# hdm0922/PathTracerDemo

Hardware: AMD Instinct MI355X
Metric: Msamples/sec at 1920x1080, 1 spp ReSTIR DI; per-pixel L2 vs WebGPU ref (higher is better)
Workload: dtype f32; 1 GPU; c3_interior_32 reuse 1920x1080, 1 spp/frame (configs[2]); frame=1920x1080, band_rows_per_gpu=1080, parallelism=row-bands x1

## Files before the change

### pathtracerdemo_amd/csrc/ptx_api.cpp

```cpp
#include <hip/hip_runtime.h>

#include <algorithm>
#include <cmath>
#include <cstdarg>
#include <cstdlib>
#include <cstdio>
#include <cstring>
#include <new>
#include <string>
#include <unordered_map>
#include <vector>

#include "ptx_internal.h"

namespace ptx {


[[maybe_unused]] static const char *const kShippedKnobs[] = {"COMM_TIMEOUT_S", "DEBUG_FILL", "HALO_PROXY_US"};
#if defined(PTX_WG_TIMES)
static const char *const kBuildKind = "wgt";
#elif defined(PTX_AB_BUILD)
static const char *const kBuildKind = "ab";
#else
static const char *const kBuildKind = "product";
// ... 37 lines not shown
            return end - pos == n ? 1 : std::atoi(ab.c_str() + pos + n + 1);
        pos = end + 1;
    }
    return dflt;
}

int fail(ptx_handle *h, int code, const char *fmt, ...) {
    if (h) {
        char buf[512];
        va_list ap;
        va_start(ap, fmt);
        vsnprintf(buf, sizeof buf, fmt, ap);
        va_end(ap);
        h->err = buf;
        gbuf_key_drop_all(h);
    }
    return code;
}
void gbuf_key_of(const ptx_handle *h, uint32_t *key) {
    static_assert(ptx_handle::kGbufKeyWords == 2 + 19 + 8 + 3, "G-buffer key words");
    key[0] = h->uniform[0];
    key[1] = h->uniform[1];
    std::memcpy(key + 2, h->uniform + 4, 19 * sizeof(uint32_t));
    std::memcpy(key + 21, h->uniform + 24, 8 * sizeof(uint32_t));
    key[29] = h->cfg.row_begin;
    key[30] = h->band_h;
    key[31] = h->halo_top;
}
void gbuf_key_drop(ptx_handle *h) { h->cur().gbuf_key_valid = false; }
void gbuf_key_drop_all(ptx_handle *h) {
    for (auto &c : h->ctx) c.gbuf_key_valid = false;
}
static bool gbuf_kept(const ptx_handle *h) {
    static const bool keep_on = ab_knob("GBUF_KEEP", 1) != 0;
    if (!keep_on || !h->cur().gbuf_key_valid || h->gbuf_exposed) return false;
    uint32_t key[ptx_handle::kGbufKeyWords];
    gbuf_key_of(h, key);
    return std::memcmp(key, h->cur().gbuf_key, sizeof key) == 0;
}
void free_buf(DevBuf &b) {
    if (b.p) (void)hipFree(b.p);
    b.p = nullptr;
    b.bytes = 0;
}
static hipError_t memset_sync(ptx_handle *h, void *p, int value, size_t bytes) {
    hipError_t e = hipMemsetAsync(p, value, bytes, h->cur().stream);
// ... 421 lines not shown
}

static size_t px_with_halo(const ptx_handle *h) {
    return (size_t)(h->halo_top + h->band_h + h->halo_bot) * h->cfg.width;
}
static uint32_t gi_job_slots(const ptx_handle *h) { return std::max(2u * h->reuse_neighbors, kGiMotionSlots); }
int reuse_buffers(ptx_handle *h) {
    const size_t njobs = (size_t)h->band_h * h->cfg.width *
                         (h->cfg.pipeline == PTX_PIPELINE_RESTIR_GI ? gi_job_slots(h) : reuse_jobs_per_px(h));
    if (h->cfg.pipeline == PTX_PIPELINE_RESTIR_GI) return alloc_buf(h, h->d_jres, njobs * 4u);
    if (int rc = alloc_buf(h, h->d_jstate, njobs * 6u * 16u)) return rc;
    if (int rc = alloc_buf(h, h->cur().nbr, px_with_halo(h) * 16u)) return rc;
    const size_t npix = (size_t)h->band_h * h->cfg.width;
    if (int rc = alloc_buf(h, h->cur().tjstate, npix * kMotionJobs * 6u * 16u)) return rc;
    if (int rc = alloc_buf(h, h->cur().tjres, npix * kMotionJobs * 16u)) return rc;
    return alloc_buf(h, h->d_jres, njobs * 16u);
}
static ReuseArgs reuse_args(ptx_handle *h, int pass) {
    ReuseArgs A{};
    A.gbuf = gbuf_band(h);
    A.cur = res_band(h);
    A.hist = hist_band(h);
    const bool temporal = pass == PTX_PASS_TEMPORAL;
    A.jstate = (float4 *)(temporal ? h->cur().tjstate.p : h->d_jstate.p);
    A.jres = (float4 *)(temporal ? h->cur().tjres.p : h->d_jres.p);
    A.jpp = temporal ? 1u : 2u * h->reuse_neighbors;
    A.njobs = h->band_h * h->cfg.width * A.jpp;
    static const bool planes = ab_knob("JOB_PLANES", 1) != 0;
    A.jpx = planes ? 1u : A.jpp;
    A.jslot = planes ? h->band_h * h->cfg.width : 1u;
    A.radius = h->reuse_radius;
    A.neighbors = h->reuse_neighbors;
    A.cap = h->temporal_cap;
    A.hist_valid = h->hist_valid && !h->hist_moved ? 1u : 0u;
    A.use_init = (pass == PTX_PASS_TEMPORAL && h->cur().init_state_valid) ? 1u : 0u;
    A.nbr_out = (uint4 *)h->cur().nbr.p + (size_t)h->halo_top * h->cfg.width;
    A.nbr = A.nbr_out;
    A.surf = h->cur().surf.p ? (const uint4 *)h->cur().surf.p + 2u * (size_t)h->halo_top * h->cfg.width : nullptr;
    static const bool fold_off = ab_knob("FOLD_LAST_STEP", 1) == 0;
    A.fold_last = ((pass == PTX_PASS_SPATIAL || pass == PTX_PASS_TEMPORAL) && !fold_off) ? 1u : 0u;
    A.ray_cap = (uint32_t)std::min<size_t>(h->cur().wave_ray_cap, 0xffffffffu);
    return A;
}

void mat4_inverse(const float *mf, float *out);
static ReuseArgs motion_args(ptx_handle *h) {
    ReuseArgs A = reuse_args(h, PTX_PASS_SPATIAL);
    A.jstate = (float4 *)h->cur().tjstate.p;
    A.jres = (float4 *)h->cur().tjres.p;
    A.jpp = kMotionJobs;
    A.njobs = h->band_h * h->cfg.width * A.jpp;
    static const bool planes = ab_knob("JOB_PLANES", 1) != 0;
    A.jpx = planes ? 1u : A.jpp;
    A.jslot = planes ? h->band_h * h->cfg.width : 1u;
    A.hist_valid = h->hist_valid ? 1u : 0u;
    A.use_init = h->cur().init_state_valid ? 1u : 0u;
    static const bool fold_on = ab_knob("FOLD_LAST_STEP", 1) != 0;
    A.fold_last = fold_on ? 1u : 0u;
    A.motion = 1u;
    std::memcpy(A.vpinv_prev, h->hist_camera, sizeof A.vpinv_prev);
    mat4_inverse(A.vpinv_prev, A.vp_prev);
    const size_t W = h->cfg.width;
    A.psurf = (const uint4 *)h->d_psurf.p + 2u * (size_t)h->halo_top * W;
    A.prev_row_lo = -(int32_t)h->halo_top;
    A.prev_row_hi = (int32_t)(h->band_h + h->halo_bot);
    A.clip = (unsigned long long *)h->d_counters.p + CNT_MOTION_CLIP;
    return A;
}

static GiArgs gi_args(ptx_handle *h, bool motion) {
    GiArgs A{};
    A.gbuf = gbuf_band(h);
    A.cur = res_band(h);
    A.hist = hist_band(h);
    A.direct = (float4 *)h->cur().direct.p;
    A.accum = (float4 *)h->d_accum.p;
    A.jray = (uint32_t *)h->d_jres.p;
    A.jpp = 2u * h->reuse_neighbors;
    static const bool planes = ab_knob("GI_JOB_PLANES", 1) != 0;
    A.jpx = planes ? 1u : A.jpp;
    A.jslot = planes ? h->band_h * h->cfg.width : 1u;
// ... 184 lines not shown
                e = wave_trace(sc, wt, r - 1, 1, h->stack_depth, st);
                event_end(t, st);
                if (e != hipSuccess) break;
            }
            if (r == nr && A.fold_last) continue;
            TimedLaunch *t = event_begin(h, PTX_STAT_WAVE_LOGIC, st);
            e = wave_reuse_round(sc, wi, 0, r, A, st);
            if (e == hipSuccess && r == 0 && halo) e = hipStreamWaitEvent(st, halo, 0);
            if (e == hipSuccess) e = wave_reuse_round(sc, we, 0, r, A, st);
            event_end(t, st);
        }
        for (const WaveBufs *ws : {&wi, &we})
            if (e == hipSuccess) e = launch_wave_seq(h, sc, *ws, PTX_PASS_FINAL, st);
    }
    if (surf_stale && e == hipSuccess) h->cur().surf_valid = true;
    return e == hipSuccess ? join_sequences(h, k) : e;
}

hipError_t launch_wave_parts(ptx_handle *h, const Scene &sc, const WaveBufs &w, const int *passes, int npasses,
                             bool summaries, const WaveBufs *then, hipEvent_t then_wait, bool keep_gbuf) {
    static const bool overlap_start = ab_knob("OVERLAP_START", 1) != 0;
    if (then && overlap_start && npasses == 2 && passes[0] == PTX_PASS_SPATIAL && passes[1] == PTX_PASS_FINAL &&
        h->cfg.pipeline == PTX_PIPELINE_RESTIR_REUSE && !summaries)
        return spatial_overlap_seq(h, sc, w, *then, then_wait);
    static const int env_k = ab_knob("WAVE_STREAMS", 0);
    static const int env_pk = ab_knob("PIPE_STREAMS", 0);
    const bool band_h = h->comm || h->halo_top || h->halo_bot || (h->cfg.flags & PTX_FLAG_HALO_SKIP);
    const int pipe_k = env_pk > 0 ? env_pk
                       : band_h || h->cfg.pipeline == PTX_PIPELINE_RESTIR_GI ||
                                 (h->cfg.pipeline == PTX_PIPELINE_RESTIR_REUSE && !reuse_static())
// ... 8 lines not shown
    k = std::max(1, std::min<int>(k, ptx_handle::kMaxSplit));
    if ((uint32_t)k > std::max(w.nseg, then ? then->nseg : 0u)) k = (int)std::max(w.nseg, then ? then->nseg : 0u);
    hipError_t e = hipSuccess;
    bool has_gbuf = false;
    for (int i = 0; i < npasses; ++i) has_gbuf |= passes[i] == PTX_PASS_GBUFFER;
    const bool skip_gbuf = has_gbuf && keep_gbuf && gbuf_kept(h);
    if (has_gbuf && !skip_gbuf) h->cur().gbuf_key_valid = false;
    for (int i = 0; i < npasses; ++i) {
        if (passes[i] == PTX_PASS_SPATIAL) {
            if (summaries && (e = spatial_summaries(h, h->cur().stream)) != hipSuccess) return e;
        } else if (passes[i] == PTX_PASS_GBUFFER && skip_gbuf) {
            continue;
        } else if (passes[i] != PTX_PASS_FINAL && passes[i] != PTX_PASS_TEMPORAL && passes[i] != kPassTemporalJobs &&
                   passes[i] != kPassTemporalCombine && !is_motion_pass(passes[i])) {
            h->cur().nbr_valid = false;
        }
    }
    bool need_surf[8] = {false};
    bool surf_ok = h->cur().surf_valid;
    for (int i = 0; i < npasses && i < 8; ++i) {
        if (passes[i] == PTX_PASS_GBUFFER) surf_ok = surf_ok && skip_gbuf;
        else if (passes[i] == PTX_PASS_INIT && w.surf) surf_ok = true;
        else if ((passes[i] == PTX_PASS_TEMPORAL || passes[i] == kPassTemporalJobs || passes[i] == PTX_PASS_SPATIAL ||
                  is_motion_pass(passes[i])) &&
                 w.surf) {
            need_surf[i] = !surf_ok;
            surf_ok = true;
        }
    }
    h->cur().surf_valid = surf_ok && w.surf;
// ... 29 lines not shown
                    e = launch_wave_seq(h, sc, part, passes[i], st);
                }
                if (e != hipSuccess) return e;
            }
        }
    }
    if ((e = join_sequences(h, k)) != hipSuccess) return e;
    if (has_gbuf && !skip_gbuf) {
        gbuf_key_of(h, h->cur().gbuf_key);
        h->cur().gbuf_key_valid = true;
    }
    for (int i = 0; i < npasses; ++i)
        if (passes[i] == PTX_PASS_TEMPORAL || passes[i] == kPassTemporalCombine || passes[i] == kPassTemporalMotion) {
            h->cur().init_state_valid = false;
            h->cur().nbr_valid = h->cfg.pipeline == PTX_PIPELINE_RESTIR_REUSE;
        }
    return hipSuccess;
}
static hipError_t launch_wave_pass(ptx_handle *h, const Scene &sc, const WaveBufs &w, int pass) {
    return launch_wave_parts(h, sc, w, &pass, 1);
}

void mark_history(ptx_handle *h) {
    std::memcpy(h->hist_camera, h->uniform + 4, sizeof h->hist_camera);
    h->hist_valid = true;
    h->hist_moved = false;
}

void mat4_inverse(const float *mf, float *out) {
    double m[16], inv[16];
// ... 181 lines not shown
        if (e == hipSuccess) e = launch_wave_parts(h, sc, w, back, 2);
        if (e == hipSuccess) mark_history(h);
    } else {
        static const int passes[3] = {PTX_PASS_GBUFFER, PTX_PASS_INIT, PTX_PASS_FINAL};
        e = launch_wave_parts(h, sc, w, passes, 3, true, nullptr, nullptr, true);
    }
    if (e != hipSuccess) return fail(h, PTX_E_HIP, "wavefront frame launch: %s", hipGetErrorString(e));
    HIP_CHECK(h, hipEventRecord(t.stop, h->cur().stream));
    t.pass = PTX_STAT_FRAME;
    t.pending = true;
    return PTX_OK;
}

static int timed_launch(ptx_handle *h, int pass) {
    if (!h->scene_loaded || !h->frame_set) return fail(h, PTX_E_INVALID, "scene and frame must be set before rendering");
    if (pass != PTX_PASS_TEMPORAL && pass != PTX_PASS_SPATIAL && pass != PTX_PASS_FINAL) h->cur().nbr_valid = false;
    if (!h->layout_valid) {
        if (int rc = build_layout(h)) return rc;
    }
    TimedLaunch &t = h->ring[h->ring_pos];
    h->ring_pos = (h->ring_pos + 1) % kEventRing;
    resolve_event(t, h);
    Scene sc = make_scene(h);
    const uint32_t fl = h->cfg.flags;
    const int variant = (fl & PTX_FLAG_SIMPLE_KERNELS) ? 2 : 3;
    WaveBufs w{};
    const bool reuse_pass = pass == PTX_PASS_TEMPORAL || pass == PTX_PASS_SPATIAL;
    if (reuse_pass && (variant != 3 || !has_reuse(h)))
        return fail(h, PTX_E_INVALID, "pass %d needs the reuse or GI pipeline (wavefront kernels)", pass);
    if (h->cfg.pipeline == PTX_PIPELINE_RESTIR_GI && pass == PTX_PASS_MCPT)
        return fail(h, PTX_E_INVALID, "the GI pipeline has no MCPT pass");
// ... 179 lines not shown
    HIP_CHECK(h, hipSetDevice(h->device));
    if (!scene || !geometry || (!accel && n_accel)) return fail(h, PTX_E_INVALID, "null scene array");
    if (int rc = quiesce(h)) return rc;
    h->scene.assign(scene, scene + n_scene);
    h->geometry.assign(geometry, geometry + n_geometry);
    h->accel.assign(accel ? accel : scene, accel ? accel + n_accel : scene);
    if (int rc = upload(h, h->d_scene, scene, n_scene * 4u)) return rc;
    if (int rc = upload(h, h->d_geometry, geometry, n_geometry * 4u)) return rc;
    h->layout_valid = false;
    h->scene_loaded = true;
    h->hist_valid = false;
    h->cur().init_state_valid = false;
    h->cur().nbr_valid = false;
    for (auto &c : h->ctx) c.surf_valid = false;
    gbuf_key_drop_all(h);
    if (h->frame_set) return build_layout(h);
    return PTX_OK;
}

int ptx_set_frame(ptx_handle *h, const uint32_t uniform[PTX_UNIFORM_WORDS]) {
    if (!h || !uniform) return PTX_E_INVALID;
    HIP_CHECK(h, hipSetDevice(h->device));
    if (uniform[0] != h->cfg.width || uniform[1] != h->cfg.height)
        return fail(h, PTX_E_INVALID, "uniform resolution %ux%u != handle %ux%u", uniform[0], uniform[1],
                    h->cfg.width, h->cfg.height);
    uint32_t key[8];
    for (int k = 0; k < 8; ++k) key[k] = uniform[24 + k];
    if (std::memcmp(key, h->layout_key, sizeof key) != 0) {
        std::memcpy(h->layout_key, key, sizeof key);
        h->layout_valid = false;
// ... 235 lines not shown
    DevBuf b;
    if (!buffer_view(h, which, b) || bytes > b.bytes)
        return fail(h, PTX_E_INVALID, "read of %zu bytes from buffer %d", bytes, which);
    if (int rc = read_to_host(h, host_dst, b.p, bytes)) return rc;
    return PTX_OK;
}

int ptx_write_buffer(ptx_handle *h, int which, const void *host_src, size_t bytes) {
    if (!h || !host_src) return PTX_E_INVALID;
    DevBuf b;
    if (!buffer_view(h, which, b) || bytes > b.bytes)
        return fail(h, PTX_E_INVALID, "write of %zu bytes to buffer %d", bytes, which);
    HIP_CHECK(h, copy_sync(h, b.p, host_src, bytes, hipMemcpyHostToDevice));
    h->cur().init_state_valid = false;
    h->cur().nbr_valid = false;
    h->cur().surf_valid = false;
    if (which == PTX_BUF_GBUFFER) gbuf_key_drop(h);
    return PTX_OK;
}

int ptx_device_pointer(ptx_handle *h, int which, void **dev_ptr, size_t *bytes) {
    if (!h || !dev_ptr) return PTX_E_INVALID;
    DevBuf b;
    if (!buffer_view(h, which, b)) return fail(h, PTX_E_INVALID, "unknown buffer %d", which);
    *dev_ptr = b.p;
    if (bytes) *bytes = b.bytes;
    if (which == PTX_BUF_GBUFFER) {
        h->gbuf_exposed = true;
        gbuf_key_drop_all(h);
    }
    return PTX_OK;
}

int ptx_present(ptx_handle *h, uint32_t canvas_w, uint32_t canvas_h, int bgra, uint8_t *out) {
    if (!h || !out) return PTX_E_INVALID;
    if (canvas_w == 0 || canvas_h == 0 || (uint64_t)canvas_w * canvas_h > (1ull << 28))
        return fail(h, PTX_E_INVALID, "ptx_present: canvas %ux%u", canvas_w, canvas_h);
    if (h->cfg.row_begin != 0 || h->band_h != h->cfg.height)
        return fail(h, PTX_E_INVALID, "ptx_present: a band handle (rows %u..%u) holds part of the texture: present the "
                                      "gathered frame on the host", h->cfg.row_begin, h->cfg.row_end);
    if (!h->d_accum.p) return fail(h, PTX_E_INVALID, "ptx_present: nothing rendered");
    HIP_CHECK(h, hipSetDevice(h->device));
    const size_t bytes = (size_t)canvas_w * canvas_h * 4u;
    if (int rc = alloc_buf(h, h->d_canvas, bytes)) return rc;
// ... 95 lines not shown
    if (h->xstream) (void)hipStreamSynchronize(h->xstream);
    comm_destroy(h);
    if (h->ctx[0].own) (void)hipStreamSynchronize(h->ctx[0].own);
    for (auto &t : h->ring) {
        if (t.start) (void)hipEventDestroy(t.start);
        if (t.stop) (void)hipEventDestroy(t.stop);
    }
    if (h->host_stage) (void)hipHostFree(h->host_stage);
    if (h->ev_present) {
        (void)hipEventSynchronize(h->ev_present);
        (void)hipEventDestroy(h->ev_present);
    }
    if (h->present_host) (void)hipHostFree(h->present_host);
    for (DevBuf *b : {&h->d_canvas, &h->d_canvas_async, &h->d_scene, &h->d_geometry, &h->d_tris, &h->d_nodes, &h->d_subs,
                      &h->d_insts, &h->d_mats, &h->d_tverts, &h->d_accum, &h->d_counters, &h->d_qrays, &h->d_qhits, &h->d_hist,
                      &h->d_jstate, &h->d_jres, &h->d_psurf, &h->d_census, &h->d_wgt})
        free_buf(*b);
    for (auto &c : h->ctx) {
        for (DevBuf *b : {&c.gbuf, &c.res, &c.direct, &c.nbr, &c.tjstate, &c.tjres, &c.surf, &c.wstate, &c.wrays, &c.wres[0],
                          &c.wres[1], &c.wres[2], &c.wact[0], &c.wact[1], &c.wctr})
            free_buf(*b);
        if (c.ev_fork) (void)hipEventDestroy(c.ev_fork);
        for (int q = 0; q < ptx_handle::kMaxSplit; ++q) {
            if (c.ev_join[q]) (void)hipEventDestroy(c.ev_join[q]);
            if (c.sub[q]) (void)hipStreamDestroy(c.sub[q]);
        }
        if (c.own) (void)hipStreamDestroy(c.own);
    }
    if (h->ev_prev) (void)hipEventDestroy(h->ev_prev);
    delete h;
    return PTX_OK;
}

const char *ptx_last_error(const ptx_handle *h) { return h ? h->err.c_str() : "null handle"; }

// ... 2 lines not shown
```

### pathtracerdemo_amd/csrc/ptx_internal.h

```cpp
#pragma once
#include <hip/hip_runtime.h>

#include <string>

#include "../../include/ptx.h"
#include "ptx_launch.h"

namespace ptx {
constexpr int kPasses = 16;
constexpr int kEventRing = 256;
struct DevBuf {
    void *p = nullptr;
    size_t bytes = 0;
};
struct TimedLaunch {
    hipEvent_t start = nullptr, stop = nullptr;
    int pass = -1;
    bool pending = false;
};
}

using namespace ptx;

constexpr int kPassTemporalJobs = 0x100, kPassTemporalCombine = 0x101;
// ... 14 lines not shown
    uint32_t layout_key[8] = {0};
    bool layout_valid = false;
    bool scene_loaded = false;
    uint32_t uniform[PTX_UNIFORM_WORDS] = {0};
    bool frame_set = false;
    uint32_t band_h = 0, halo_top = 0, halo_bot = 0;
    DevBuf d_accum, d_counters, d_hist, d_jstate, d_jres;
    uint32_t res_u4 = 8;
    bool gbuf_exposed = false;
    uint32_t reuse_radius = 0, reuse_neighbors = 0, temporal_cap = 0;
    float4 *mcpt_color = nullptr;
    bool hist_valid = false;
    uint32_t hist_camera[19] = {0};
    bool hist_moved = false;
    DevBuf d_psurf;
    DevBuf d_qrays, d_qhits;
    DevBuf d_census;
    uint32_t census_blocks = 0;
    DevBuf d_wgt;
    static constexpr int kMaxCtx = 3;
    static constexpr int kMaxSplit = 4;
    static constexpr int kGbufKeyWords = 32;
    struct FrameCtx {
        DevBuf gbuf, res, direct;
        DevBuf nbr, tjstate, tjres;
        DevBuf surf;
        DevBuf wstate, wrays, wres[3], wact[2], wctr;
        size_t wave_ray_cap = 0;
        hipStream_t own = nullptr, stream = nullptr;
        hipStream_t sub[kMaxSplit] = {nullptr, nullptr, nullptr, nullptr};
        hipEvent_t ev_fork = nullptr, ev_join[kMaxSplit] = {nullptr, nullptr, nullptr, nullptr};
        bool init_state_valid = false;
        bool nbr_valid = false;
        bool surf_valid = false;
        uint32_t gbuf_key[kGbufKeyWords] = {0};
        bool gbuf_key_valid = false;
    } ctx[kMaxCtx];
    int ctx_idx = 0;
    FrameCtx &cur() { return ctx[ctx_idx]; }
    const FrameCtx &cur() const { return ctx[ctx_idx]; }
    hipEvent_t ev_prev = nullptr;
    void *comm = nullptr;
    int rank = 0, world = 1;
    hipStream_t xstream = nullptr;
    hipEvent_t ev_front = nullptr, ev_halo = nullptr;
    hipEvent_t ev_mhalo = nullptr;
    uint64_t halo_bytes_sent = 0;
    bool comm_broken = false;
    uint64_t band_frames = 0;
    uint32_t band_camera[19] = {0};
    DevBuf d_canvas;
// ... 24 lines not shown
int read_to_host(ptx_handle *h, void *dst, const void *src, size_t bytes);
uint4 *gbuf_band(ptx_handle *h);
uint4 *res_band(ptx_handle *h);
bool has_reuse(const ptx_handle *h);
int build_layout(ptx_handle *h);
Scene make_scene(ptx_handle *h);
void resolve_event(TimedLaunch &t, ptx_handle *h);
int wave_buffers(ptx_handle *h, WaveBufs &w);
int reuse_buffers(ptx_handle *h);
hipError_t launch_wave_parts(ptx_handle *h, const Scene &sc, const WaveBufs &w, const int *passes, int npasses,
                             bool summaries = true, const WaveBufs *then = nullptr, hipEvent_t then_wait = nullptr,
                             bool keep_gbuf = false);
void gbuf_key_of(const ptx_handle *h, uint32_t *key);
void gbuf_key_drop(ptx_handle *h);
void gbuf_key_drop_all(ptx_handle *h);
hipError_t spatial_summaries(ptx_handle *h, hipStream_t st);
void mark_history(ptx_handle *h);
int motion_prepare(ptx_handle *h, hipStream_t st);
uint4 *hist_band(ptx_handle *h);
bool pipelined(const ptx_handle *h);
int quiesce(ptx_handle *h);
int pipe_depth();
int ensure_contexts(ptx_handle *h);
void next_frame_ctx(ptx_handle *h);
int first_frame_ctx(ptx_handle *h);
int render_band_nccl(ptx_handle *h);
int render_band_solo(ptx_handle *h);
void comm_destroy(ptx_handle *h);
const char *comm_library();
}
// ... 1 lines not shown
```

### pathtracerdemo_amd/csrc/ptx_launch.h

```cpp
#pragma once

#include <hip/hip_runtime.h>

#include "ptx_device.h"

namespace ptx {

constexpr int kTile = 16;
constexpr int kBlock = 256;

int env_knob(const char *key, int dflt);
#ifdef PTX_AB_BUILD
inline int ab_knob(const char *key, int dflt) { return env_knob(key, dflt); }
#else
constexpr int ab_knob(const char *, int dflt) { return dflt; }
#endif

inline size_t stack_lds_bytes(uint32_t depth) { return (size_t)depth * kBlock * sizeof(uint32_t); }

hipError_t launch_gbuffer(const Scene &sc, uint4 *gbuf, uint32_t stack_depth, hipStream_t s);
hipError_t launch_init(const Scene &sc, const uint4 *gbuf, uint4 *reservoir, uint32_t stack_depth, hipStream_t s);
hipError_t launch_final(const Scene &sc, const uint4 *gbuf, const uint4 *reservoir, float4 *accum,
                        uint32_t stack_depth, hipStream_t s);
hipError_t launch_mcpt(const Scene &sc, float4 *accum, uint32_t stack_depth, hipStream_t s);
// ... 58 lines not shown
    float4 *jres;
    uint32_t njobs, jpp;
    uint32_t jpx, jslot;
    uint32_t radius, neighbors, cap, hist_valid;
    uint32_t use_init;
    const uint4 *nbr;
    uint4 *nbr_out;
    const uint4 *surf;
    uint32_t fold_last;
    uint32_t ray_cap;
    uint32_t motion;
    float vpinv_prev[16], vp_prev[16];
    const uint4 *psurf;
    int32_t prev_row_lo, prev_row_hi;
    unsigned long long *clip;
};
constexpr uint32_t kMotionJobs = 3u;
constexpr uint32_t kJobPending = 0xFFFFFFFFu;
static_assert(kWaveRoundsReuse <= 3, "fold_last: one result buffer per reuse trace round");
int reuse_rounds(int pass_temporal, const ReuseArgs &A);
hipError_t wave_reuse_round(const Scene &sc, const WaveBufs &w, int pass_temporal, int round, const ReuseArgs &A,
                            hipStream_t s);
hipError_t wave_reuse_summary(const Scene &sc, const uint4 *gbuf, const uint4 *res, uint4 *nbr, uint4 *surf,
                              size_t npx, hipStream_t s);
hipError_t wave_surface(const Scene &sc, const WaveBufs &w, const uint4 *gbuf, hipStream_t s);

constexpr int kWaveRoundsGiInit = 2, kWaveRoundsGiSpatial = 1;
constexpr uint32_t kGiResU4 = 4u;
struct GiArgs {
    const uint4 *gbuf;
// ... 18 lines not shown
```

### pathtracerdemo_amd/csrc/ptx_reuse.hip

```cpp
#include "ptx_wave_common.h"

namespace ptx {

constexpr uint32_t SALT_TEMPORAL = 0x54454D50u, SALT_SPATIAL = 0x53504154u;

enum : uint32_t { JS_HDR, JS_F, JS_CUR, JS_NRM, JS_PREV, JS_RRF, JS_COUNT };
constexpr uint32_t kJobFresh = 1u << 24;
constexpr uint32_t kResReuseLayout = 0x100u;
#ifndef PTX_JOB_FRESH
#define PTX_JOB_FRESH 1
#endif

struct Job {
    uint32_t i, length, phase, seed1, idx, matref;
    uint32_t k, lab;
    bool shift, rok;
    int32_t ref;
    int32_t dom;
    f3 f;
    float prod;
    Surface cur;
    f3 prev;
    float beta, rr_p;
    f3 rr_f;
};

__device__ __forceinline__ uint32_t job_id(const ReuseArgs &A, uint32_t pix, uint32_t slot) {
    return pix * A.jpx + slot * A.jslot;
}
__device__ __forceinline__ const uint4 *res_at(const uint4 *base, int32_t idx) { return base + 8 * (ptrdiff_t)idx; }
constexpr int32_t kHistRef = 1 << 30;
__device__ __forceinline__ const uint4 *res_of(const ReuseArgs &A, int32_t ref) {
    return ref >= (kHistRef >> 1) ? A.hist + 8 * (ptrdiff_t)(ref - kHistRef) : A.cur + 8 * (ptrdiff_t)ref;
}
constexpr int32_t kDomPrev = INT32_MIN;

__device__ __forceinline__ uint32_t job_hw(const Job &s) {
    return s.i | (s.length << 8) | (s.phase << 16) | (s.lab << 18) | (s.rok ? 1u << 21 : 0u) |
           (s.shift ? 1u << 22 : 0u) | (s.k << 25);
}
__device__ __forceinline__ void job_unhw(Job &s, uint32_t hw) {
    s.i = hw & 0xffu; s.length = (hw >> 8) & 0xffu; s.phase = (hw >> 16) & 3u;
    s.lab = (hw >> 18) & 7u; s.rok = (hw >> 21) & 1u; s.shift = (hw >> 22) & 1u; s.k = (hw >> 25) & 7u;
}
__device__ __forceinline__ void job_store(const ReuseArgs &A, uint32_t jid, const Job &s) {
    const size_t n = A.njobs;
    float4 *st = A.jstate;
    if (PTX_JOB_FRESH && s.i == 1u && s.phase == 0u && s.dom != kDomPrev) {
// ... 92 lines not shown
}
__device__ __forceinline__ float rc_geo(f3 prev, const Surface &Xk) {
    const f3 dv = Xk.pos - prev;
    const float d2 = dot(dv, dv);
    const float ck = fabsf(dot(Xk.nrm, dv / __builtin_sqrtf(d2)));
    return d2 / ck;
}
__device__ __forceinline__ uint4 rc_next(const uint4 *rv, uint32_t w20) {
    return (w20 & kResReuseLayout) ? rv[0] : rv[6];
}

enum : int { JK_ANY = -1, JK_L = 0, JK_C = 1, JK_B = 2 };
__device__ __forceinline__ int job_kind(uint32_t length, uint32_t k) {
    return length <= 2u ? JK_L : (k == 2u ? JK_C : JK_B);
}
template <int KIND = JK_ANY>
__device__ __forceinline__ bool job_emit(const Scene &sc, const Seg &g, const ReuseArgs &A, bool emit, Job &s,
                                         uint32_t jid, uint32_t seed0) {
    bool ray = false, vis = false, go = false;
    f3 o = mk(0.0f, 0.0f, 0.0f), d = o, Le = o;
    float remain = -1.0f;
    if (emit) {
        const uint4 *rv = res_of(A, s.ref);
        const f3 V = normalize(s.prev - s.cur.pos);
        const bool hyb = job_hyb(s);
        bool ok = true;
        if (KIND == JK_ANY ? s.i + 1u < s.length : KIND != JK_L) {
            const bool conn = KIND == JK_ANY ? s.shift && hyb && s.i + 1u == s.k : KIND == JK_C;
            const bool fixd = KIND == JK_ANY && s.shift && hyb && s.i == s.k;
            f3 dir;
            uint32_t lobe = LOBE_LAMBERT;
            if (conn || fixd) {
                const uint4 r5 = rv[5];
                const Surface Xt = get_surface(sc, gdecode(conn ? rv[4] : rc_next(rv, r5.x)));
                if (conn) {
                    const bool rk1 = rough_under(s.cur, r5.y), rk = rough_under(Xt, r5.z);
                    if (s.i >= 2u && s.lab == 0u && safe_edge(s.rok, rk1, s.prev, s.cur.pos)) s.lab = s.i;
// ... 35 lines not shown
            const f3 L = direction_to_light(s.cur, XL);
            if (XL.type == LIGHT_ENV) {
                float pdf;
                const f3 fv = bsdf_pdf(s.cur, V, L, pdf);
                ok = rr_step(s, s.cur, L, fv, pdf) && ok;
            }
            s.f = s.f * (bsdf(s.cur, L, V) * fabsf(dot(s.cur.nrm, L)));
            float gl = 1.0f;
            if (XL.type == LIGHT_RECT) {
                const f3 r = XL.pos - s.cur.pos;
                const f3 Ld = normalize(r);
                gl = fabsf(dot(get_light(sc, (uint32_t)XL.id).dir, Ld)) / dot(r, r);
            }
            s.prod = hyb ? s.prod / s.beta : s.prod / (gl * s.beta);
            Le = l_emit<true>(XL, s.cur);
            s.phase = 1u;
            const float dist = length(XL.pos - s.cur.pos);
            o = s.cur.pos; d = (XL.pos - s.cur.pos) / dist; remain = dist;
            vis = true;
            ray = go = ok;
        }
        if (!go) A.jres[jid] = make_float4(0.0f, 0.0f, 0.0f, 0.0f);
    }
    const uint32_t idx = g.rbase + wave_alloc(g.l_ray, ray ? 1u : 0u);
    if (ray) {
        s.idx = idx;
        put_ray(g.rays, idx, o, d, remain, vis ? Q_VIS : Q_CLOSEST);
        if (vis) g.res_out[2u * idx] = make_float4(0.0f, Le.x, Le.y, Le.z);
    }
    return go;
}

__device__ __forceinline__ void job_finish(const Seg &g, const JobLists &JL, const ReuseArgs &A, bool live,
                                           const Job &s, uint32_t jid) {
    if (live) job_store(A, jid, s);
    const bool fold = live && A.fold_last && s.phase == 1u;
    if (fold) A.jres[jid] = make_float4(asf(s.idx), asf(g.out_sel), 0.0f, asf(kJobPending));
// ... 48 lines not shown
                        s.prod = s.prod * rc_geo(s.cur.pos, next);
                    s.prev = s.cur.pos;
                    s.cur = next;
                    s.matref = nref;
                    s.i += 1u;
                    emit = true;
                }
            } else {
                const float4 a = g.res_in[2u * s.idx];
                s.f = s.f * (mk(a.y, a.z, a.w) * a.x);
                const float qv = s.prod;
                const bool valid = qv > 0.0f && qv <= 3.402823466e38f;
                A.jres[jid] = valid ? make_float4(s.f.x, s.f.y, s.f.z, qv) : make_float4(0.0f, 0.0f, 0.0f, 0.0f);
            }
        }
        const bool live = job_emit(sc, g, A, emit, s, jid, 0u);
        job_finish(g, JL, A, live, s, jid);
    }
    job_seg_end(w, g, JL);
    return *g.l_ray;
}
__global__ __launch_bounds__(WB) __attribute__((amdgpu_waves_per_eu(JOB_STEP_WAVES, 8)))
void wjob_step(Scene sc, WaveBufs w, uint32_t round, ReuseArgs A) {
    PTX_WAVE_TIMER(sc, KID_JOB_STEP | (w.seg_base ? 0x80u : 0u));
    __shared__ uint32_t lds[3];
    (void)job_step_segment(sc, w, round, A, lds);
}

__device__ __forceinline__ uint32_t reuse_seed(const Scene &sc, uint32_t x, uint32_t y, uint32_t salt) {
    return pcg(pcg(x * 1973u + y * 9277u + sc.U[U_FRAME] * 26699u) ^ salt);
}
// ... 99 lines not shown
        const uint32_t q = seg_pixel(w, g.j, k);
        uint32_t x, y, pix = 0u;
        bool active = false;
        Job s;
        if (q < np && tile_xy(sc, q, x, y)) {
            pix = (y - sc.row_begin) * sc.width + x;
            active = job_begin(sc, A, s, x, y, (int32_t)pix, (int32_t)pix);
            if (active && A.use_init) active = temporal_from_init(sc, w, A, s, pix, pix);
        }
        const bool live = job_emit(sc, g, A, active, s, pix, active ? A.cur[8u * (size_t)pix].x : 0u);
        job_finish(g, JL, A, live, s, pix);
    }
    job_seg_end(w, g, JL);
}

__global__ __launch_bounds__(WB) void wtemporal_combine(Scene sc, WaveBufs w, ReuseArgs A) {
    PTX_WAVE_TIMER(sc, KID_TEMP_COMBINE | (w.seg_base ? 0x80u : 0u));
    const uint32_t j = w.seg_base + blockIdx.x, np = padded_pixels(sc);
    for (uint32_t k = 0; k < w.seg_px; k += WB) {
        const uint32_t q = seg_pixel(w, j, k);
        uint32_t x, y;
        if (q >= np || !tile_xy(sc, q, x, y)) continue;
        const uint32_t pix = (y - sc.row_begin) * sc.width + x;
        if (!gdecode(A.gbuf[pix]).valid) {
            A.nbr_out[pix] = make_uint4(0u, 0u, 0u, 0u);
            continue;
        }
        uint4 *rv = A.cur + 8u * (size_t)pix;
        const uint4 *hv = A.hist + 8u * (size_t)pix;
        uint32_t seed = reuse_seed(sc, x, y, SALT_TEMPORAL);
        const uint4 r5 = rv[5], r7 = rv[7];
        const float4 er = (r7.y != 0u && r5.w >= 2u) ? job_result(A, w, A.jres[pix], pix) : make_float4(0.0f, 0.0f, 0.0f, 0.0f);
        const float2 ec = make_float2(er.w > 0.0f ? luminance(mk(er.x, er.y, er.z)) : 0.0f, er.w);
        const bool canon_ok = ec.y > 0.0f && ec.x > 0.0f;
        const uint4 h5 = hv[5], h6 = hv[6], h7 = hv[7];
        const uint32_t Cp = A.hist_valid ? min(h7.y, A.cap) : 0u;
        const float cp = (float)Cp, tot = 1.0f + cp;
        const float pp = asf(h6.x), qp = asf(h6.y);
        const bool hist_ok = Cp != 0u && h5.w >= 2u && pp > 0.0f;
        const float wc = canon_ok ? (1.0f / tot) * ec.x * asf(r7.x) : 0.0f;
        const float wp = hist_ok ? (cp / tot) * pp * asf(h7.x) : 0.0f;
        float w_sum = 0.0f, p_sel = ec.x, q_sel = ec.y;
        bool from_hist = false;
        if (wrs_update(w_sum, wc, seed)) { from_hist = false; p_sel = ec.x; q_sel = ec.y; }
        if (wrs_update(w_sum, wp, seed)) { from_hist = true; p_sel = pp; q_sel = qp; }
        write_reused(rv, from_hist ? hv : rv, p_sel, q_sel, from_hist ? stored_f(hv) : job_f(er), w_sum, 1u + Cp);
        const float W = p_sel > 0.0f ? w_sum / p_sel : 0.0f;
        A.nbr_out[pix] = nbr_pack(true, make_uint4(from_hist ? h5.x : r5.x, 0u, 0u, from_hist ? h5.w : r5.w),
                                  make_uint4(asu(p_sel), asu(q_sel), 0u, 0u), make_uint4(asu(W), 1u + Cp, 0u, 0u));
    }
}

__device__ __forceinline__ f3 x0_prev(const ReuseArgs &A, const Scene &sc, uint32_t x, uint32_t y) {
    float u = ((float)x + 0.5f) / (float)sc.U[U_W];
    float v = ((float)y + 0.5f) / (float)sc.U[U_H];
    return xform_point(A.vpinv_prev, mk(2.0f * u - 1.0f, 2.0f * v - 1.0f, 0.0f));
}
struct MotionHist { bool ok; int32_t pp; uint32_t px, py, C; };
__device__ __forceinline__ MotionHist motion_hist(const Scene &sc, const ReuseArgs &A, const Surface &X1, uint32_t y,
                                                  bool count = false) {
    MotionHist m{false, 0, 0u, 0u, 0u};
// ... 90 lines not shown
    job_seg_end(w, g, JL);
}

__global__ __launch_bounds__(WB) void wtmotion_combine(Scene sc, WaveBufs w, ReuseArgs A) {
    PTX_WAVE_TIMER(sc, KID_TEMP_COMBINE | (w.seg_base ? 0x80u : 0u));
    const uint32_t j = w.seg_base + blockIdx.x, np = padded_pixels(sc);
    for (uint32_t k = 0; k < w.seg_px; k += WB) {
        const uint32_t q = seg_pixel(w, j, k);
        uint32_t x, y;
        if (q >= np || !tile_xy(sc, q, x, y)) continue;
        const uint32_t pix = (y - sc.row_begin) * sc.width + x;
        Surface X1;
        uint32_t mref;
        if (!surf_load(sc, A.surf, pix, X1, mref)) {
            A.nbr_out[pix] = make_uint4(0u, 0u, 0u, 0u);
            continue;
        }
        uint4 *rv = A.cur + 8u * (size_t)pix;
        uint32_t seed = reuse_seed(sc, x, y, SALT_TEMPORAL);
        const uint4 r5 = rv[5], r7 = rv[7];
        const float4 er = (r7.y != 0u && r5.w >= 2u) ? job_at(A, w, pix, 0u) : make_float4(0.0f, 0.0f, 0.0f, 0.0f);
        const float ecp = er.w > 0.0f ? luminance(mk(er.x, er.y, er.z)) : 0.0f, ecq = er.w;
        const bool canon_ok = ecq > 0.0f && ecp > 0.0f;
        const float cc = 1.0f, pc = ecp, qc = ecq, Wc = asf(r7.x);
        const MotionHist mh = motion_hist(sc, A, X1, y);
        const uint32_t Cp = mh.ok ? mh.C : 0u;
        const float cp = (float)Cp;
        const uint4 *hv = A.hist + 8 * (ptrdiff_t)mh.pp;
        float wh = 0.0f, pf = 0.0f, qf = 0.0f;
        SelF ff{false, mk(0.0f, 0.0f, 0.0f)};
// ... 21 lines not shown
        float Q = 1.0f;
        if (canon_ok && Cp != 0u) {
            const float4 B = job_at(A, w, pix, 2u);
            if (B.w > 0.0f) {
                const float pbc = luminance(mk(B.x, B.y, B.z)) * qc / B.w;
                const float den = cc * pc + cp * pbc;
                Q = den > 0.0f ? (cc * pc) / den : 1.0f;
            }
        }
        const float wc = canon_ok ? Q * pc * Wc : 0.0f;
        float w_sum = 0.0f, p_sel = ecp, q_sel = ecq;
        bool from_hist = false;
        if (wrs_update(w_sum, wc, seed)) { from_hist = false; p_sel = ecp; q_sel = ecq; }
        if (wrs_update(w_sum, wh, seed)) { from_hist = true; p_sel = pf; q_sel = qf; }
        write_reused(rv, from_hist ? hv : rv, p_sel, q_sel, from_hist ? ff : job_f(er), w_sum, 1u + Cp);
        const float Wo = p_sel > 0.0f ? w_sum / p_sel : 0.0f;
        A.nbr_out[pix] = nbr_pack(true, make_uint4(from_hist ? hk : r5.x, 0u, 0u, from_hist ? hlen : r5.w),
                                  make_uint4(asu(p_sel), asu(q_sel), 0u, 0u), make_uint4(asu(Wo), 1u + Cp, 0u, 0u));
    }
}

__device__ __forceinline__ bool spatial_neighbor(uint32_t &seed, uint32_t R, uint32_t x, uint32_t y, uint32_t W,
                                                 uint32_t H, uint32_t &nx, uint32_t &ny) {
    const float side = (float)(2u * R + 1u);
    uint32_t ix = (uint32_t)(rnd(seed) * side);
    uint32_t iy = (uint32_t)(rnd(seed) * side);
    ix = min(ix, 2u * R);
    iy = min(iy, 2u * R);
    const int X = (int)x + (int)ix - (int)R, Y = (int)y + (int)iy - (int)R;
    if (X < 0 || Y < 0 || X >= (int)W || Y >= (int)H || (ix == R && iy == R)) return false;
// ... 295 lines not shown
        if (wrs_update(w_sum, wc, seed)) { src = (int32_t)pix; p_sel = c.pc; q_sel = c.qc; f_sel = stored_f(rc); }
        for (uint32_t m = 0; m < M; ++m) {
            uint32_t nx = 0u, ny = 0u;
            float wn = 0.0f, pf = 0.0f, qf = 0.0f;
            SelF fj{false, mk(0.0f, 0.0f, 0.0f)};
            int32_t nidx = 0;
            if (spatial_neighbor(nseed, A.radius, x, y, sc.width, sc.height, nx, ny)) {
                nidx = band_index(sc, nx, ny);
                wn = neighbour_weight(c, Mf, nbr_at(A, nidx), job_at(A, w, pix, 2u * m), pf,
                                      qf, fj);
            }
            if (wrs_update(w_sum, wn, seed)) { src = nidx; p_sel = pf; q_sel = qf; f_sel = fj; }
        }
    }
    write_reused(out, res_at(A.cur, src), p_sel, q_sel, f_sel, w_sum, Csum);
}

constexpr uint32_t kShflLanes = 4u;
__global__ __launch_bounds__(WB) void wspatial_combine_shfl(Scene sc, WaveBufs w, ReuseArgs A) {
    PTX_WAVE_TIMER(sc, KID_SPAT_COMBINE | (w.seg_base ? 0x80u : 0u));
    constexpr uint32_t M = 3u;
    const uint32_t j = w.seg_base + blockIdx.x, np = padded_pixels(sc);
    const uint32_t lane = __lane_id(), r = lane & 3u, base = lane & ~3u;
    for (uint32_t k = 0; k < w.seg_px; k += WB / kShflLanes) {
        const uint32_t off = k + (threadIdx.x >> 2), sl = off >> 6;
        const uint32_t q = set_tile(w, ((sl / w.cluster) * w.nseg + j) * w.cluster + sl % w.cluster) * 64u + (off & 63u);
        uint32_t x = 0u, y = 0u;
        const bool inside = q < np && tile_xy(sc, q, x, y);
        const uint32_t pix = inside ? (y - sc.row_begin) * sc.width + x : 0u;
        const bool hit = inside && gdecode(A.gbuf[pix]).valid;
// ... 35 lines not shown
        w_sum += w0; if (r == 0u) w_upto = w_sum;
        w_sum += w1; if (r == 1u) w_upto = w_sum;
        w_sum += w2; if (r == 2u) w_upto = w_sum;
        w_sum += w3; if (r == 3u) w_upto = w_sum;
        uint32_t dseed = seed0 + 2u * M + r;
        const bool accept = hit && rnd(dseed) < wn / w_upto;
        const uint32_t grp = (uint32_t)(__ballot(accept) >> base) & 0xfu;
        const uint32_t sel = grp ? 31u - (uint32_t)__builtin_clz(grp) : 0u;
        const int32_t src_l = r == 0u ? (int32_t)pix : (pres ? nid : 0);
        const int32_t src = __shfl(src_l, base + sel);
        const float p_sel = sel ? __shfl(pf, base + sel) : c.pc, q_sel = sel ? __shfl(qf, base + sel) : c.qc;
        const float fx = __shfl(fj.f.x, base + sel), fy = __shfl(fj.f.y, base + sel), fz = __shfl(fj.f.z, base + sel);
        const bool fk = __shfl(fj.known ? 1 : 0, base + sel) != 0;
        if (!inside) continue;
        uint4 *out = A.hist + 8u * (size_t)pix;
        if (!hit) {
            out[2u * r] = make_uint4(0u, 0u, 0u, 0u);
            out[2u * r + 1u] = make_uint4(0u, 0u, 0u, 0u);
            continue;
        }
        if (r < 3u) {
            const uint4 *sv = res_at(A.cur, src);
            const uint4 a0 = sv[2u * r], a1 = sv[2u * r + 1u];
            out[2u * r] = a0;
            out[2u * r + 1u] = a1;
        } else {
            const SelF fs = sel ? SelF{fk, mk(fx, fy, fz)} : stored_f(A.cur + 8u * (size_t)pix);
            out[6] = make_uint4(asu(p_sel), asu(q_sel), fs.known ? asu(fs.f.x) : 0u, fs.known ? asu(fs.f.y) : 0u);
            out[7] = make_uint4(asu(p_sel > 0.0f ? w_sum / p_sel : 0.0f), Csum, fs.known ? asu(fs.f.z) : 0u,
                                fs.known ? 1u : 0u);
        }
    }
}

__global__ __launch_bounds__(WB) void wspatial_combine(Scene sc, WaveBufs w, ReuseArgs A) {
    PTX_WAVE_TIMER(sc, KID_SPAT_COMBINE | (w.seg_base ? 0x80u : 0u));
    const uint32_t j = w.seg_base + blockIdx.x, np = padded_pixels(sc);
    for (uint32_t k = 0; k < w.seg_px; k += WB) {
        const uint32_t q = seg_pixel(w, j, k);
        uint32_t x, y;
        if (q >= np || !tile_xy(sc, q, x, y)) continue;
        const uint32_t pix = (y - sc.row_begin) * sc.width + x;
        if (!gdecode(A.gbuf[pix]).valid) {
            uint4 *out = A.hist + 8u * (size_t)pix;
            for (int t = 0; t < 8; ++t) out[t] = make_uint4(0u, 0u, 0u, 0u);
            continue;
        }
        if (A.neighbors == 3u) combine_pixel<3>(sc, A, w, x, y, pix);
        else combine_pixel<0>(sc, A, w, x, y, pix);
    }
}

int reuse_rounds(int pass_temporal, const ReuseArgs &A) {
    return pass_temporal && A.use_init && !A.motion ? 1 : kWaveRoundsReuse;
}

hipError_t wave_reuse_round(const Scene &sc, const WaveBufs &w, int pass_temporal, int round, const ReuseArgs &A,
                            hipStream_t s) {
    const dim3 grid(w.seg_count), blk(WB);
    if (round == 0) {
// ... 17 lines not shown
```

Measured before the change: 568.7 Msamples/s.

## Cache per-reservoir light visibility to skip shadow rays in reuse shift jobs

Adds per-pixel visibility buffers (current and history) that record the visibility term of each selected reservoir sample, written by the temporal and spatial combine kernels. During reuse job emission, hybrid shift jobs look up the cached visibility of the source reservoir and write the final contribution directly instead of tracing a shadow ray. This removes shadow-ray tracing work at the cost of extra per-pixel stores and loads, plus invalidation bookkeeping. Reusing a source's visibility at a shifted path vertex may be an approximation if the visibility actually differs.

```diff
diff --git a/pathtracerdemo_amd/csrc/ptx_api.cpp b/pathtracerdemo_amd/csrc/ptx_api.cpp
--- a/pathtracerdemo_amd/csrc/ptx_api.cpp
+++ b/pathtracerdemo_amd/csrc/ptx_api.cpp
@@ -75,6 +75,7 @@
         va_end(ap);
         h->err = buf;
         gbuf_key_drop_all(h);
+        tvis_drop_all(h);
     }
     return code;
 }
@@ -91,6 +92,10 @@
 void gbuf_key_drop(ptx_handle *h) { h->cur().gbuf_key_valid = false; }
 void gbuf_key_drop_all(ptx_handle *h) {
     for (auto &c : h->ctx) c.gbuf_key_valid = false;
+}
+void tvis_drop_all(ptx_handle *h) {
+    for (auto &c : h->ctx) c.tvis_valid = false;
+    h->tvis_hist_valid = false;
 }
 static bool gbuf_kept(const ptx_handle *h) {
     static const bool keep_on = ab_knob("GBUF_KEEP", 1) != 0;
@@ -542,6 +547,12 @@
     const size_t npix = (size_t)h->band_h * h->cfg.width;
     if (int rc = alloc_buf(h, h->cur().tjstate, npix * kMotionJobs * 6u * 16u)) return rc;
     if (int rc = alloc_buf(h, h->cur().tjres, npix * kMotionJobs * 16u)) return rc;
+    if (!h->halo_top && !h->halo_bot && h->band_h == h->cfg.height) {
+        if (!h->cur().tvis.p) h->cur().tvis_valid = false;
+        if (int rc = alloc_buf(h, h->cur().tvis, npix * 4u)) return rc;
+        if (!h->d_tvis_hist.p) h->tvis_hist_valid = false;
+        if (int rc = alloc_buf(h, h->d_tvis_hist, npix * 4u)) return rc;
+    }
     return alloc_buf(h, h->d_jres, njobs * 16u);
 }
 static ReuseArgs reuse_args(ptx_handle *h, int pass) {
@@ -568,6 +579,12 @@
     static const bool fold_off = ab_knob("FOLD_LAST_STEP", 1) == 0;
     A.fold_last = ((pass == PTX_PASS_SPATIAL || pass == PTX_PASS_TEMPORAL) && !fold_off) ? 1u : 0u;
     A.ray_cap = (uint32_t)std::min<size_t>(h->cur().wave_ray_cap, 0xffffffffu);
+    static const bool tvis_on = ab_knob("TVIS_KEEP", 1) != 0;
+    const bool rd = tvis_on && !h->res_exposed && h->cur().tvis.p && h->d_tvis_hist.p;
+    A.tv_cur = rd && !temporal && h->cur().tvis_valid ? (const float *)h->cur().tvis.p : nullptr;
+    A.tv_hist = rd && h->tvis_hist_valid ? (const float *)h->d_tvis_hist.p : nullptr;
+    A.tv_out = (float *)(temporal ? h->cur().tvis.p : h->d_tvis_hist.p);
+    A.tv_cur_stride = 1u;
     return A;
 }
 
@@ -593,6 +610,12 @@
     A.prev_row_lo = -(int32_t)h->halo_top;
     A.prev_row_hi = (int32_t)(h->band_h + h->halo_bot);
     A.clip = (unsigned long long *)h->d_counters.p + CNT_MOTION_CLIP;
+    static const bool tvis_on = ab_knob("TVIS_KEEP", 1) != 0;
+    const bool init = tvis_on && !h->res_exposed && A.tv_out && A.use_init && h->cur().wstate.p;
+    A.tv_cur = init ? (const float *)((const float4 *)h->cur().wstate.p + (size_t)kStateTsel * h->band_h * h->cfg.width)
+                    : nullptr;
+    A.tv_cur_stride = 4u;
+    A.tv_out = (float *)h->cur().tvis.p;
     return A;
 }
 
@@ -807,6 +830,7 @@
             if (e == hipSuccess) e = launch_wave_seq(h, sc, *ws, PTX_PASS_FINAL, st);
     }
     if (surf_stale && e == hipSuccess) h->cur().surf_valid = true;
+    if (e == hipSuccess) h->tvis_hist_valid = A.tv_out != nullptr;
     return e == hipSuccess ? join_sequences(h, k) : e;
 }
 
@@ -845,6 +869,7 @@
         } else if (passes[i] != PTX_PASS_FINAL && passes[i] != PTX_PASS_TEMPORAL && passes[i] != kPassTemporalJobs &&
                    passes[i] != kPassTemporalCombine && !is_motion_pass(passes[i])) {
             h->cur().nbr_valid = false;
+            h->cur().tvis_valid = false;
         }
     }
     bool need_surf[8] = {false};
@@ -904,6 +929,9 @@
         if (passes[i] == PTX_PASS_TEMPORAL || passes[i] == kPassTemporalCombine || passes[i] == kPassTemporalMotion) {
             h->cur().init_state_valid = false;
             h->cur().nbr_valid = h->cfg.pipeline == PTX_PIPELINE_RESTIR_REUSE;
+            h->cur().tvis_valid = h->cur().nbr_valid && h->cur().tvis.p;
+        } else if (passes[i] == PTX_PASS_SPATIAL && h->cfg.pipeline == PTX_PIPELINE_RESTIR_REUSE) {
+            h->tvis_hist_valid = h->d_tvis_hist.p != nullptr;
         }
     return hipSuccess;
 }
@@ -1115,7 +1143,8 @@
 
 static int timed_launch(ptx_handle *h, int pass) {
     if (!h->scene_loaded || !h->frame_set) return fail(h, PTX_E_INVALID, "scene and frame must be set before rendering");
-    if (pass != PTX_PASS_TEMPORAL && pass != PTX_PASS_SPATIAL && pass != PTX_PASS_FINAL) h->cur().nbr_valid = false;
+    if (pass != PTX_PASS_TEMPORAL && pass != PTX_PASS_SPATIAL && pass != PTX_PASS_FINAL)
+        h->cur().nbr_valid = h->cur().tvis_valid = false;
     if (!h->layout_valid) {
         if (int rc = build_layout(h)) return rc;
     }
@@ -1325,6 +1354,7 @@
     h->cur().nbr_valid = false;
     for (auto &c : h->ctx) c.surf_valid = false;
     gbuf_key_drop_all(h);
+    tvis_drop_all(h);
     if (h->frame_set) return build_layout(h);
     return PTX_OK;
 }
@@ -1590,6 +1620,8 @@
     HIP_CHECK(h, copy_sync(h, b.p, host_src, bytes, hipMemcpyHostToDevice));
     h->cur().init_state_valid = false;
     h->cur().nbr_valid = false;
+    h->cur().tvis_valid = false;
+    if (which == PTX_BUF_RESERVOIR_HIST) h->tvis_hist_valid = false;
     h->cur().surf_valid = false;
     if (which == PTX_BUF_GBUFFER) gbuf_key_drop(h);
     return PTX_OK;
@@ -1604,6 +1636,10 @@
     if (which == PTX_BUF_GBUFFER) {
         h->gbuf_exposed = true;
         gbuf_key_drop_all(h);
+    }
+    if (which == PTX_BUF_RESERVOIR || which == PTX_BUF_RESERVOIR_HIST) {
+        h->res_exposed = true;
+        tvis_drop_all(h);
     }
     return PTX_OK;
 }
@@ -1729,11 +1765,11 @@
     if (h->present_host) (void)hipHostFree(h->present_host);
     for (DevBuf *b : {&h->d_canvas, &h->d_canvas_async, &h->d_scene, &h->d_geometry, &h->d_tris, &h->d_nodes, &h->d_subs,
                       &h->d_insts, &h->d_mats, &h->d_tverts, &h->d_accum, &h->d_counters, &h->d_qrays, &h->d_qhits, &h->d_hist,
-                      &h->d_jstate, &h->d_jres, &h->d_psurf, &h->d_census, &h->d_wgt})
+                      &h->d_jstate, &h->d_jres, &h->d_psurf, &h->d_census, &h->d_wgt, &h->d_tvis_hist})
         free_buf(*b);
     for (auto &c : h->ctx) {
         for (DevBuf *b : {&c.gbuf, &c.res, &c.direct, &c.nbr, &c.tjstate, &c.tjres, &c.surf, &c.wstate, &c.wrays, &c.wres[0],
-                          &c.wres[1], &c.wres[2], &c.wact[0], &c.wact[1], &c.wctr})
+                          &c.wres[1], &c.wres[2], &c.wact[0], &c.wact[1], &c.wctr, &c.tvis})
             free_buf(*b);
         if (c.ev_fork) (void)hipEventDestroy(c.ev_fork);
         for (int q = 0; q < ptx_handle::kMaxSplit; ++q) {
diff --git a/pathtracerdemo_amd/csrc/ptx_internal.h b/pathtracerdemo_amd/csrc/ptx_internal.h
--- a/pathtracerdemo_amd/csrc/ptx_internal.h
+++ b/pathtracerdemo_amd/csrc/ptx_internal.h
@@ -52,6 +52,8 @@
     uint32_t hist_camera[19] = {0};
     bool hist_moved = false;
     DevBuf d_psurf;
+    DevBuf d_tvis_hist;
+    bool tvis_hist_valid = false, res_exposed = false;
     DevBuf d_qrays, d_qhits;
     DevBuf d_census;
     uint32_t census_blocks = 0;
@@ -73,6 +75,8 @@
         bool surf_valid = false;
         uint32_t gbuf_key[kGbufKeyWords] = {0};
         bool gbuf_key_valid = false;
+        DevBuf tvis;
+        bool tvis_valid = false;
     } ctx[kMaxCtx];
     int ctx_idx = 0;
     FrameCtx &cur() { return ctx[ctx_idx]; }
@@ -127,6 +131,7 @@
 void gbuf_key_of(const ptx_handle *h, uint32_t *key);
 void gbuf_key_drop(ptx_handle *h);
 void gbuf_key_drop_all(ptx_handle *h);
+void tvis_drop_all(ptx_handle *h);
 hipError_t spatial_summaries(ptx_handle *h, hipStream_t st);
 void mark_history(ptx_handle *h);
 int motion_prepare(ptx_handle *h, hipStream_t st);
diff --git a/pathtracerdemo_amd/csrc/ptx_launch.h b/pathtracerdemo_amd/csrc/ptx_launch.h
--- a/pathtracerdemo_amd/csrc/ptx_launch.h
+++ b/pathtracerdemo_amd/csrc/ptx_launch.h
@@ -96,6 +96,9 @@
     const uint4 *psurf;
     int32_t prev_row_lo, prev_row_hi;
     unsigned long long *clip;
+    const float *tv_cur, *tv_hist;
+    float *tv_out;
+    uint32_t tv_cur_stride;
 };
 constexpr uint32_t kMotionJobs = 3u;
 constexpr uint32_t kJobPending = 0xFFFFFFFFu;
diff --git a/pathtracerdemo_amd/csrc/ptx_reuse.hip b/pathtracerdemo_amd/csrc/ptx_reuse.hip
--- a/pathtracerdemo_amd/csrc/ptx_reuse.hip
+++ b/pathtracerdemo_amd/csrc/ptx_reuse.hip
@@ -32,6 +32,13 @@
 constexpr int32_t kHistRef = 1 << 30;
 __device__ __forceinline__ const uint4 *res_of(const ReuseArgs &A, int32_t ref) {
     return ref >= (kHistRef >> 1) ? A.hist + 8 * (ptrdiff_t)(ref - kHistRef) : A.cur + 8 * (ptrdiff_t)ref;
+}
+__device__ __forceinline__ float tvis_cur(const ReuseArgs &A, int32_t idx) {
+    return A.tv_cur ? A.tv_cur[(ptrdiff_t)idx * (ptrdiff_t)A.tv_cur_stride] : -1.0f;
+}
+__device__ __forceinline__ float tvis_of(const ReuseArgs &A, int32_t ref) {
+    if (ref < (kHistRef >> 1)) return tvis_cur(A, ref);
+    return A.tv_hist ? A.tv_hist[ref - kHistRef] : -1.0f;
 }
 constexpr int32_t kDomPrev = INT32_MIN;
 
@@ -154,13 +161,14 @@
 __device__ __forceinline__ int job_kind(uint32_t length, uint32_t k) {
     return length <= 2u ? JK_L : (k == 2u ? JK_C : JK_B);
 }
-template <int KIND = JK_ANY>
+template <int KIND = JK_ANY, bool KEEP = false>
 __device__ __forceinline__ bool job_emit(const Scene &sc, const Seg &g, const ReuseArgs &A, bool emit, Job &s,
                                          uint32_t jid, uint32_t seed0) {
     bool ray = false, vis = false, go = false;
     f3 o = mk(0.0f, 0.0f, 0.0f), d = o, Le = o;
     float remain = -1.0f;
     if (emit) {
+        float4 done = make_float4(0.0f, 0.0f, 0.0f, 0.0f);
         const uint4 *rv = res_of(A, s.ref);
         const f3 V = normalize(s.prev - s.cur.pos);
         const bool hyb = job_hyb(s);
@@ -226,13 +234,23 @@
             }
             s.prod = hyb ? s.prod / s.beta : s.prod / (gl * s.beta);
             Le = l_emit<true>(XL, s.cur);
+            if (KEEP && s.shift && hyb && ok) {
+                const float T = tvis_of(A, s.ref);
+                if (T >= 0.0f) {
+                    const f3 f = s.f * (Le * T);
+                    const float qv = s.prod;
+                    const bool valid = qv > 0.0f && qv <= 3.402823466e38f;
+                    if (valid) done = make_float4(f.x, f.y, f.z, qv);
+                    ok = false;
+                }
+            }
             s.phase = 1u;
             const float dist = length(XL.pos - s.cur.pos);
             o = s.cur.pos; d = (XL.pos - s.cur.pos) / dist; remain = dist;
             vis = true;
             ray = go = ok;
         }
-        if (!go) A.jres[jid] = make_float4(0.0f, 0.0f, 0.0f, 0.0f);
+        if (!go) A.jres[jid] = done;
     }
     const uint32_t idx = g.rbase + wave_alloc(g.l_ray, ray ? 1u : 0u);
     if (ray) {
@@ -311,7 +329,7 @@
                 A.jres[jid] = valid ? make_float4(s.f.x, s.f.y, s.f.z, qv) : make_float4(0.0f, 0.0f, 0.0f, 0.0f);
             }
         }
-        const bool live = job_emit(sc, g, A, emit, s, jid, 0u);
+        const bool live = job_emit<JK_ANY, true>(sc, g, A, emit, s, jid, 0u);
         job_finish(g, JL, A, live, s, jid);
     }
     job_seg_end(w, g, JL);
@@ -441,6 +459,12 @@
     job_seg_end(w, g, JL);
 }
 
+__device__ __forceinline__ float tvis_temporal(const WaveBufs &w, const ReuseArgs &A, uint32_t pix, bool from_hist,
+                                               int32_t hp) {
+    if (from_hist) return A.tv_hist ? A.tv_hist[hp] : -1.0f;
+    return A.use_init ? w.state[kStateTsel * w.npix + pix].x : -1.0f;
+}
+
 __global__ __launch_bounds__(WB) void wtemporal_combine(Scene sc, WaveBufs w, ReuseArgs A) {
     PTX_WAVE_TIMER(sc, KID_TEMP_COMBINE | (w.seg_base ? 0x80u : 0u));
     const uint32_t j = w.seg_base + blockIdx.x, np = padded_pixels(sc);
@@ -451,6 +475,7 @@
         const uint32_t pix = (y - sc.row_begin) * sc.width + x;
         if (!gdecode(A.gbuf[pix]).valid) {
             A.nbr_out[pix] = make_uint4(0u, 0u, 0u, 0u);
+            if (A.tv_out) A.tv_out[pix] = -1.0f;
             continue;
         }
         uint4 *rv = A.cur + 8u * (size_t)pix;
@@ -472,6 +497,7 @@
         if (wrs_update(w_sum, wc, seed)) { from_hist = false; p_sel = ec.x; q_sel = ec.y; }
         if (wrs_update(w_sum, wp, seed)) { from_hist = true; p_sel = pp; q_sel = qp; }
         write_reused(rv, from_hist ? hv : rv, p_sel, q_sel, from_hist ? stored_f(hv) : job_f(er), w_sum, 1u + Cp);
+        if (A.tv_out) A.tv_out[pix] = tvis_temporal(w, A, pix, from_hist, (int32_t)pix);
         const float W = p_sel > 0.0f ? w_sum / p_sel : 0.0f;
         A.nbr_out[pix] = nbr_pack(true, make_uint4(from_hist ? h5.x : r5.x, 0u, 0u, from_hist ? h5.w : r5.w),
                                   make_uint4(asu(p_sel), asu(q_sel), 0u, 0u), make_uint4(asu(W), 1u + Cp, 0u, 0u));
@@ -592,6 +618,7 @@
         uint32_t mref;
         if (!surf_load(sc, A.surf, pix, X1, mref)) {
             A.nbr_out[pix] = make_uint4(0u, 0u, 0u, 0u);
+            if (A.tv_out) A.tv_out[pix] = -1.0f;
             continue;
         }
         uint4 *rv = A.cur + 8u * (size_t)pix;
@@ -643,6 +670,7 @@
         if (wrs_update(w_sum, wc, seed)) { from_hist = false; p_sel = ecp; q_sel = ecq; }
         if (wrs_update(w_sum, wh, seed)) { from_hist = true; p_sel = pf; q_sel = qf; }
         write_reused(rv, from_hist ? hv : rv, p_sel, q_sel, from_hist ? ff : job_f(er), w_sum, 1u + Cp);
+        if (A.tv_out) A.tv_out[pix] = tvis_temporal(w, A, pix, from_hist, mh.pp);
         const float Wo = p_sel > 0.0f ? w_sum / p_sel : 0.0f;
         A.nbr_out[pix] = nbr_pack(true, make_uint4(from_hist ? hk : r5.x, 0u, 0u, from_hist ? hlen : r5.w),
                                   make_uint4(asu(p_sel), asu(q_sel), 0u, 0u), make_uint4(asu(Wo), 1u + Cp, 0u, 0u));
@@ -968,6 +996,7 @@
         }
     }
     write_reused(out, res_at(A.cur, src), p_sel, q_sel, f_sel, w_sum, Csum);
+    if (A.tv_out) A.tv_out[pix] = tvis_cur(A, src);
 }
 
 constexpr uint32_t kShflLanes = 4u;
@@ -1033,6 +1062,7 @@
         const bool fk = __shfl(fj.known ? 1 : 0, base + sel) != 0;
         if (!inside) continue;
         uint4 *out = A.hist + 8u * (size_t)pix;
+        if (r == 0u && A.tv_out) A.tv_out[pix] = hit ? tvis_cur(A, src) : -1.0f;
         if (!hit) {
             out[2u * r] = make_uint4(0u, 0u, 0u, 0u);
             out[2u * r + 1u] = make_uint4(0u, 0u, 0u, 0u);
@@ -1063,6 +1093,7 @@
         if (!gdecode(A.gbuf[pix]).valid) {
             uint4 *out = A.hist + 8u * (size_t)pix;
             for (int t = 0; t < 8; ++t) out[t] = make_uint4(0u, 0u, 0u, 0u);
+            if (A.tv_out) A.tv_out[pix] = -1.0f;
             continue;
         }
         if (A.neighbors == 3u) combine_pixel<3>(sc, A, w, x, y, pix);
```

Result: no change. 563.8 Msamples/s (-0.9%).
